# Superjomn/TiPS

Measured on AMD Instinct MI355X. Metric: device-resident fp32 bucket-sum GiB/s (% HBM peak); allreduce GiB/s 1/2/4/8 GPU, higher is better.
Workload: dtype f32

## Files before the change

### tips_amd/csrc/mxfp8.cc

```cpp
#include <algorithm>
#include <vector>

#include "mxfp8.h"
#include "rt.h"
#include "side.h"

using namespace tips::rt;

namespace {

const char kTakes[] = "the MXFP8 calls take";

struct Flat {
  int64_t elems = 0, total = 0;
  std::vector<tips::MxSeg> segs;
};

int flat_of(const void* const* ptrs, const int64_t* counts, int n, bool cover, Flat* f) {
  if (n > 0 && !ptrs) return fail(TIPS_ERR_INVALID_ARG, "bad tensor list (n %d)", n);
  TRY(check_counts(counts, n, "tensor", &f->total));
  if (f->total == 0) return 0;
  std::vector<int64_t> offs((size_t)n);
  f->elems = fused_layout(counts, n, TIPS_FLOAT32, offs.data()) / 4;
  for (int i = 0; i < n; i++)
    if (counts[i] > 0) {
      if (!ptrs[i]) return fail(TIPS_ERR_INVALID_ARG, "null pointer (tensor %d)", i);
      if ((reinterpret_cast<uintptr_t>(ptrs[i]) & 3) != 0) return fail(TIPS_ERR_INVALID_ARG, "tensor %d is not 4-B aligned", i);
      f->segs.push_back(tips::MxSeg{ptrs[i], offs[i] / 4, counts[i], (counts[i] + 31) / 32 * 32});
    }
  std::sort(f->segs.begin(), f->segs.end(), [](const tips::MxSeg& a, const tips::MxSeg& b) { return a.off < b.off; });
  if (cover) tips::mxfp8_cover(f->segs, tips::mxfp8_scales_offset(f->elems));
  return 0;
}
// ... 5 lines not shown
}

int quantize_into(const Flat& f, unsigned char* wire, float* residual, hipStream_t s) {
  const int64_t so = tips::mxfp8_scales_offset(f.elems);
  const int64_t tail_begin = so / tips::kMxBlock, tail_end = tips::mxfp8_wire_bytes(f.elems) - so;
  HIP_TRY(tips::launch_mxfp8_quantize(f.segs.data(), (int)f.segs.size(), wire, wire + so, residual, tail_begin, tail_end, s));
  return 0;
}

int64_t ef_sender_elems(int64_t E) { return tips::mxfp8_scales_offset(E); }
int64_t ef_elems(int64_t E, int p) {
  const int64_t per = p > 1 ? chunk_of(tips::mxfp8_blocks(E), p, 8, 0).len() : 0;
  return ef_sender_elems(E) + tips::kMxBlock * per;
}

bool overlaps(const void* a, int64_t an, const void* b, int64_t bn) {
  const uintptr_t x = reinterpret_cast<uintptr_t>(a), y = reinterpret_cast<uintptr_t>(b);
  return an > 0 && bn > 0 && x < y + (uintptr_t)bn && y < x + (uintptr_t)an;
}

int check_residual(const void* r, int64_t bytes, const char* what, const Flat* a, const Flat* b) {
  TRY(need_device(r, what, kTakes));
  if ((reinterpret_cast<uintptr_t>(r) & 15) != 0) return fail(TIPS_ERR_INVALID_ARG, "%s must be 16-B aligned", what);
  for (const Flat* f : {a, b})
    if (f)
      for (const tips::MxSeg& sg : f->segs)
        if (sg.ptr && overlaps(r, bytes, sg.ptr, sg.count * 4)) return fail(TIPS_ERR_INVALID_ARG, "%s overlaps a tensor of the list", what);
  return 0;
}

int dequantize_from(const Flat& f, const unsigned char* wire, double factor, hipStream_t s) {
  HIP_TRY(tips::launch_mxfp8_dequantize(f.segs.data(), (int)f.segs.size(), wire, wire + tips::mxfp8_scales_offset(f.elems),
                                        (float)factor, s));
  return 0;
}

int at_most_max_srcs(const char* what, int size) {
  if (size > tips::kMxMaxSrcs)
    return fail(TIPS_ERR_UNSUPPORTED, "%s folds at most %d ranks, not %d", what, tips::kMxMaxSrcs, size);
  return 0;
}

int agree(int size, int n, int64_t total, const int64_t* counts, int own, bool with_ef) {
  const uint64_t h = hash_counts(counts, n);
  const int64_t mine[4] = {n, total, (int64_t)(with_ef ? (h ^ 0xEFull) * kFnvPrime : h), own};
  SideRecords rec;
  TRY(side_exchange(size, mine, 4, &rec));
  if (const int r = rec.first_differing(0, 3); r >= 0) {
    const int64_t *q = rec.of(r), *q0 = rec.of(0);
    return fail(TIPS_ERR_MISMATCH,
                "Mismatched MXFP8 allreduce: rank %d has %lld tensors, %lld elements, count hash %llx; rank 0 has %lld "
                "tensors, %lld elements, count hash %llx",
                r, (long long)q[0], (long long)q[1], (unsigned long long)q[2], (long long)q0[0], (long long)q0[1],
                (unsigned long long)q0[2]);
  }
  if (!own) TRY(rec.report_refusing("MXFP8 allreduce"));
  return rec.report_own();
}

struct Part {
  unsigned char *payload, *scales;
  int64_t blocks;
};

template <class To, class From>
int exchange(State& st, hipStream_t s, To&& to, From&& from) {
  TRY(rccl_enter(st, s));
  NCCL_TRY(ncclGroupStart());
  for (int q = 0; q < st.size; q++) {
    if (q == st.rank) continue;
    const Part t = to(q), f = from(q);
    if (t.blocks > 0) {
      NCCL_TRY(ncclSend(t.payload, (size_t)(t.blocks * tips::kMxBlock), ncclInt8, q, st.comm, s));
      NCCL_TRY(ncclSend(t.scales, (size_t)t.blocks, ncclInt8, q, st.comm, s));
    }
    if (f.blocks > 0) {
      NCCL_TRY(ncclRecv(f.payload, (size_t)(f.blocks * tips::kMxBlock), ncclInt8, q, st.comm, s));
      NCCL_TRY(ncclRecv(f.scales, (size_t)f.blocks, ncclInt8, q, st.comm, s));
    }
  }
  NCCL_TRY(ncclGroupEnd());
  return rccl_leave(st, s);
}

int run_collective(State& st, const Flat& in, const Flat& out, double factor, float* ef, hipStream_t s) {
  const int p = st.size, rank = st.rank;
  const int64_t E = in.elems, B = tips::mxfp8_blocks(E), so = tips::mxfp8_scales_offset(E);
  const int64_t wire = tips::mxfp8_wire_bytes(E);
  const int64_t per = p > 1 ? chunk_of(B, p, 8, 0).len() : 0;
  const int64_t slot = round_up(per * tips::kMxBlock + per, kAlignBytes);
  TRY(st.mxfp8.open(s, (size_t)(2 * wire + (p - 1) * slot)));
  unsigned char* w0 = (unsigned char*)st.mxfp8.scratch.p;
  unsigned char* w1 = w0 + wire;
  unsigned char* stage = w1 + wire;
  TRY(quantize_into(in, w0, ef, s));
  const unsigned char* reduced = w0;
  if (p > 1) {
    TRY(ensure_comm(st));
    auto slot_of = [&](int r) { return stage + (int64_t)(r < rank ? r : r - 1) * slot; };
    auto staged = [&](int r, int64_t blocks) { return Part{slot_of(r), slot_of(r) + per * tips::kMxBlock, blocks}; };
    auto blocks_of = [&](unsigned char* w, Range c) { return Part{w + c.b * tips::kMxBlock, w + so + c.b, c.len()}; };
    const Range mine = chunk_of(B, p, 8, rank);
    TRY(exchange(
        st, s, [&](int q) { return blocks_of(w0, chunk_of(B, p, 8, q)); }, [&](int q) { return staged(q, mine.len()); }));
    if (mine.len() > 0) {
      tips::MxSrcs srcs = {};
      for (int r = 0; r < p; r++) {
        const Part src = r == rank ? blocks_of(w0, mine) : staged(r, mine.len());
        srcs.payload[r] = src.payload;
        srcs.scales[r] = src.scales;
      }
      const Part dst = blocks_of(w1, mine);
      HIP_TRY(tips::launch_mxfp8_fold(dst.payload, dst.scales, srcs, p, mine.len(), ef ? ef + ef_sender_elems(E) : nullptr, s));
    }
    TRY(exchange(
        st, s, [&](int) { return blocks_of(w1, mine); }, [&](int q) { return blocks_of(w1, chunk_of(B, p, 8, q)); }));
    reduced = w1;
  }
  TRY(dequantize_from(out, reduced, factor, s));
  return st.mxfp8.close(s);
}

int collective(const char* what, const void* const* ins, const int64_t* counts, int n, void* const* outs, double factor,
               bool with_ef, void* ef, int64_t ef_bytes, hipStream_t s) {
  TRY(check_factor(factor));
  Flat in, out;
  TRY(flat_of(ins, counts, n, true, &in));
  TRY(flat_of(outs, counts, n, false, &out));
  State& st = S();
  std::unique_lock<std::mutex> one;
  int size;
  TRY(side_open(st, st.mxfp8, what, "MXFP8", at_most_max_srcs, true, &one, &size));
  int own = refuse_capture(what, s);
  for (size_t i = 0; i < in.segs.size() && own == 0; i++)
    if (in.segs[i].ptr) own = need_device(in.segs[i].ptr, "an input", kTakes);
  for (size_t i = 0; i < out.segs.size() && own == 0; i++) own = need_device(out.segs[i].ptr, "an output", kTakes);
  if (with_ef && in.total > 0 && own == 0) {
    const int64_t need = 4 * ef_elems(in.elems, size);
    if (ef_bytes < need)
      own = fail(TIPS_ERR_MISMATCH, "%s: ef_bytes %lld is below tips_mxfp8_ef_bytes(%lld, %d) = %lld", what, (long long)ef_bytes,
                 (long long)in.elems, size, (long long)need);
    else own = check_residual(ef, need, "ef", &in, &out);
  }
  TRY(agree(size, n, in.total, counts, own, with_ef));
  if (in.total == 0) return 0;
  std::lock_guard<std::mutex> lk(st.mu);
  if (!st.initialized) return fail(TIPS_ERR_NOT_INITIALIZED, "tips_init has not been called");
  TRY(set_device(st));
  return run_collective(st, in, out, factor, with_ef ? (float*)ef : nullptr, s);
}

int fold_blocks(void* dst_wire, const void* const* src_wires, int nsrc, int64_t flat_elems, int64_t block_begin,
                int64_t block_count, bool with_ef, void* residual, hipStream_t s) {
  if (nsrc < 1 || nsrc > tips::kMxMaxSrcs) return fail(TIPS_ERR_INVALID_ARG, "nsrc must be 1 ... %d (got %d)", tips::kMxMaxSrcs, nsrc);
  if (flat_elems < 0 || flat_elems > ((int64_t)1 << 56) || block_begin < 0 || block_count < 0)
    return fail(TIPS_ERR_INVALID_ARG, "negative size (elements %lld, blocks %lld + %lld)", (long long)flat_elems,
                (long long)block_begin, (long long)block_count);
  if (block_count > tips::mxfp8_blocks(flat_elems) - block_begin)
    return fail(TIPS_ERR_INVALID_ARG, "blocks %lld + %lld lie outside the buffer's %lld", (long long)block_begin,
                (long long)block_count, (long long)tips::mxfp8_blocks(flat_elems));
  if (!src_wires) return fail(TIPS_ERR_INVALID_ARG, "null pointer (src_wires)");
  if (block_count == 0) return 0;
  TRY(check_wire(dst_wire, "dst_wire"));
  const int64_t so = tips::mxfp8_scales_offset(flat_elems);
  tips::MxSrcs srcs = {};
  for (int j = 0; j < nsrc; j++) {
    TRY(check_wire(src_wires[j], "a source wire buffer"));
    srcs.payload[j] = (const unsigned char*)src_wires[j] + block_begin * tips::kMxBlock;
    srcs.scales[j] = (const unsigned char*)src_wires[j] + so + block_begin;
  }
  if (with_ef) {
    const int64_t rbytes = 4 * tips::kMxBlock * block_count, wbytes = tips::mxfp8_wire_bytes(flat_elems);
    TRY(check_residual(residual, rbytes, "residual", nullptr, nullptr));
    bool hit = overlaps(residual, rbytes, dst_wire, wbytes);
    for (int j = 0; j < nsrc; j++) hit = hit || overlaps(residual, rbytes, src_wires[j], wbytes);
    if (hit) return fail(TIPS_ERR_INVALID_ARG, "residual overlaps a wire buffer");
  }
  unsigned char* d = (unsigned char*)dst_wire;
  HIP_TRY(tips::launch_mxfp8_fold(d + block_begin * tips::kMxBlock, d + so + block_begin, srcs, nsrc, block_count,
                                  with_ef ? (float*)residual : nullptr, s));
  return 0;
}

int flat_collective(const char* what, const void* const* ins, const int64_t* counts, int n, void* flat, double factor,
                    bool with_ef, void* ef, int64_t ef_bytes, hipStream_t s) {
  if (n < 0 || (n > 0 && (!counts || !ins))) return fail(TIPS_ERR_INVALID_ARG, "bad tensor list (n %d)", n);
  std::vector<int64_t> offs((size_t)n);
  std::vector<void*> outs((size_t)n, nullptr);
  int64_t total;
  TRY(check_counts(counts, n, "tensor", &total));
  if (total > 0) {
    if (!flat) return fail(TIPS_ERR_INVALID_ARG, "null pointer (flat)");
    fused_layout(counts, n, TIPS_FLOAT32, offs.data());
    for (int i = 0; i < n; i++)
      if (counts[i] > 0) outs[i] = (char*)flat + offs[i];
  }
  return collective(what, ins, counts, n, outs.data(), factor, with_ef, ef, ef_bytes, s);
}

}

extern "C" {

int64_t tips_mxfp8_wire_bytes(int64_t flat_elems, int64_t* scales_offset) {
  if (flat_elems < 0 || flat_elems > ((int64_t)1 << 56)) return fail(TIPS_ERR_INVALID_ARG, "bad size (%lld elements)", (long long)flat_elems);
  if (scales_offset) *scales_offset = tips::mxfp8_scales_offset(flat_elems);
  return tips::mxfp8_wire_bytes(flat_elems);
}

int tips_mxfp8_quantize(const void* const* ins, const int64_t* counts, int n, void* wire, void* stream) {
  Flat f;
  TRY(flat_of(ins, counts, n, true, &f));
  if (f.total == 0) return 0;
  TRY(check_wire(wire, "wire"));
  for (const tips::MxSeg& sg : f.segs)
    if (sg.ptr) TRY(need_device(sg.ptr, "a tensor of the list", kTakes));
  return quantize_into(f, (unsigned char*)wire, nullptr, (hipStream_t)stream);
}

int64_t tips_mxfp8_ef_bytes(int64_t flat_elems, int nranks) {
  if (flat_elems < 0 || flat_elems > ((int64_t)1 << 56)) return fail(TIPS_ERR_INVALID_ARG, "bad size (%lld elements)", (long long)flat_elems);
  if (nranks < 1 || nranks > tips::kMxMaxSrcs) return fail(TIPS_ERR_INVALID_ARG, "nranks must be 1 ... %d (got %d)", tips::kMxMaxSrcs, nranks);
  return 4 * ef_elems(flat_elems, nranks);
}

int tips_mxfp8_quantize_ef(const void* const* ins, const int64_t* counts, int n, void* wire, void* residual, void* stream) {
  Flat f;
  TRY(flat_of(ins, counts, n, true, &f));
  if (f.total == 0) return 0;
  TRY(check_wire(wire, "wire"));
  for (const tips::MxSeg& sg : f.segs)
    if (sg.ptr) TRY(need_device(sg.ptr, "a tensor of the list", kTakes));
  const int64_t rbytes = 4 * ef_sender_elems(f.elems);
  TRY(check_residual(residual, rbytes, "residual", &f, nullptr));
  if (overlaps(residual, rbytes, wire, tips::mxfp8_wire_bytes(f.elems))) return fail(TIPS_ERR_INVALID_ARG, "residual overlaps the wire buffer");
  return quantize_into(f, (unsigned char*)wire, (float*)residual, (hipStream_t)stream);
}

int tips_mxfp8_fold(void* dst_wire, const void* const* src_wires, int nsrc, int64_t flat_elems, int64_t block_begin,
                    int64_t block_count, void* stream) {
  return fold_blocks(dst_wire, src_wires, nsrc, flat_elems, block_begin, block_count, false, nullptr, (hipStream_t)stream);
}

int tips_mxfp8_fold_ef(void* dst_wire, const void* const* src_wires, int nsrc, int64_t flat_elems, int64_t block_begin,
                       int64_t block_count, void* residual, void* stream) {
  return fold_blocks(dst_wire, src_wires, nsrc, flat_elems, block_begin, block_count, true, residual, (hipStream_t)stream);
}

int tips_mxfp8_dequantize(void* const* outs, const int64_t* counts, int n, const void* wire, double factor, void* stream) {
  TRY(check_factor(factor));
  Flat f;
  TRY(flat_of(outs, counts, n, false, &f));
  if (f.total == 0) return 0;
  TRY(check_wire(wire, "wire"));
  for (const tips::MxSeg& sg : f.segs) TRY(need_device(sg.ptr, "a tensor of the list", kTakes));
  return dequantize_from(f, (const unsigned char*)wire, factor, (hipStream_t)stream);
}

int tips_allreduce_mxfp8(const void* in, void* out, int64_t count, double factor, void* stream) {
  if (count < 0) return fail(TIPS_ERR_INVALID_ARG, "negative count");
  return collective("tips_allreduce_mxfp8", &in, &count, 1, &out, factor, false, nullptr, 0, (hipStream_t)stream);
}

int tips_allreduce_mxfp8_ef(const void* in, void* out, int64_t count, double factor, void* ef, int64_t ef_bytes, void* stream) {
  if (count < 0) return fail(TIPS_ERR_INVALID_ARG, "negative count");
  return collective("tips_allreduce_mxfp8_ef", &in, &count, 1, &out, factor, true, ef, ef_bytes, (hipStream_t)stream);
}

int tips_fused_allreduce_mxfp8_flat(const void* const* ins, const int64_t* counts, int n, void* flat, double factor,
                                    void* stream) {
  return flat_collective("tips_fused_allreduce_mxfp8_flat", ins, counts, n, flat, factor, false, nullptr, 0, (hipStream_t)stream);
}

int tips_fused_allreduce_mxfp8_ef_flat(const void* const* ins, const int64_t* counts, int n, void* flat, double factor,
                                       void* ef, int64_t ef_bytes, void* stream) {
  return flat_collective("tips_fused_allreduce_mxfp8_ef_flat", ins, counts, n, flat, factor, true, ef, ef_bytes,
                         (hipStream_t)stream);
}

}
```

### tips_amd/csrc/mxfp8.h

```cpp
#pragma once

#include <hip/hip_runtime.h>
#include <stdint.h>

#include <vector>

namespace tips {

constexpr int kMxBlock = 32;
inline int64_t mxfp8_blocks(int64_t elems) { return (elems + kMxBlock - 1) / kMxBlock; }
inline int64_t mxfp8_scales_offset(int64_t elems) { return (elems + 255) / 256 * 256; }
inline int64_t mxfp8_wire_bytes(int64_t elems) { return mxfp8_scales_offset(elems) + (mxfp8_blocks(elems) + 255) / 256 * 256; }

struct MxSeg {
  const void* ptr;
  int64_t off, count, span;
};
constexpr int kMxSegsPerLaunch = 48;
constexpr int64_t kMxTileElems = 4096;

inline void mxfp8_cover(std::vector<MxSeg>& segs, int64_t end) {
  for (size_t i = 0; i < segs.size(); i++) segs[i].span = (i + 1 < segs.size() ? segs[i + 1].off : end) - segs[i].off;
  if (segs[0].off > 0) segs.insert(segs.begin(), MxSeg{nullptr, 0, 0, segs[0].off});
}

hipError_t launch_mxfp8_quantize(const MxSeg* segs, int nseg, unsigned char* payload, unsigned char* scales,
                                 float* residual, int64_t tail_begin, int64_t tail_end, hipStream_t s);
constexpr int kMxMaxSrcs = 16;
struct MxSrcs {
  const unsigned char* payload[kMxMaxSrcs];
  const unsigned char* scales[kMxMaxSrcs];
};
hipError_t launch_mxfp8_fold(unsigned char* dst_payload, unsigned char* dst_scales, const MxSrcs& srcs, int nsrc,
                             int64_t nblocks, float* residual, hipStream_t s);
hipError_t launch_mxfp8_dequantize(const MxSeg* segs, int nseg, const unsigned char* payload, const unsigned char* scales,
                                   float factor, hipStream_t s);

struct MxFoldSeg {
  const void* own;
  void* dst;
  int64_t off, count;
};
constexpr int kMxFoldSegsPerLaunch = 80;
hipError_t launch_mxfp8_fold_segs(const MxFoldSeg* segs, int nseg, const MxSrcs& wires, int nsrc, int own_pos, float factor,
                                  hipStream_t s);

}
```

### tips_amd/csrc/mxfp8.hip

```cpp
#include <type_traits>
#include <vector>

#include "kernels_device.h"
#include "mxfp8.h"
#include "reducescatter.h"

namespace tips {

namespace {

constexpr int kMxRounds = 4;
static_assert(kMxTileElems == (int64_t)kBlock * kMxRounds * 4, "a tile is 256 lanes x 4 rounds x 4 elements");
constexpr unsigned kInfBits = 0x7f800000u, kQuietNaN = 0x7fc00000u, kMax448 = 0x43e00000u;

typedef short s16x2 __attribute__((ext_vector_type(2)));
typedef float f32x2 __attribute__((ext_vector_type(2)));

struct MxSegList {
  MxSeg seg[kMxSegsPerLaunch];
  int64_t tile0[kMxSegsPerLaunch + 1];
  int nseg;
};

__device__ __forceinline__ unsigned max8(unsigned v) {
// ... 16 lines not shown
__device__ __forceinline__ float scaled_clamped(float x, float mul) {
#pragma clang fp contract(off)
  const unsigned b = __builtin_bit_cast(unsigned, x * mul);
  return __builtin_bit_cast(float, min(b & 0x7fffffffu, kMax448) | (b & 0x80000000u));
}

__device__ __forceinline__ unsigned encode4(f32x4 x, unsigned sb) {
  const float mul = __builtin_bit_cast(float, (254u - sb) << 23);
  int w = __builtin_amdgcn_cvt_pk_fp8_f32(scaled_clamped(x[0], mul), scaled_clamped(x[1], mul), 0, false);
  w = __builtin_amdgcn_cvt_pk_fp8_f32(scaled_clamped(x[2], mul), scaled_clamped(x[3], mul), w, true);
  return (unsigned)w;
}

__device__ __forceinline__ unsigned abs_max4(f32x4 x) {
  const u32x4 b = __builtin_bit_cast(u32x4, x) & 0x7fffffffu;
  return max(max(b[0], b[1]), max(b[2], b[3]));
}

__device__ __forceinline__ float scale_value(unsigned sb) {
  return __builtin_bit_cast(float, sb == 255u ? kQuietNaN : (sb ? (sb << 23) : 0x00400000u));
}

template <class List>
__device__ __forceinline__ int seg_of_tile(const List& L, int64_t t) {
  int lo = 0, hi = L.nseg - 1;
  while (lo < hi) {
    const int mid = (lo + hi + 1) >> 1;
    if (L.tile0[mid] <= t) lo = mid;
    else hi = mid - 1;
  }
  return lo;
}

template <bool HI>
__device__ __forceinline__ f32x2 decode2(unsigned w, float scale) {
#pragma clang fp contract(off)
  return __builtin_amdgcn_cvt_pk_f32_fp8((int)w, HI) * scale;
}

__device__ __forceinline__ f32x4 residual4(f32x4 c, unsigned w, unsigned sb) {
#pragma clang fp contract(off)
  const float scale = scale_value(sb);
  const f32x2 lo = decode2<false>(w, scale), hi = decode2<true>(w, scale);
  return f32x4{c[0] - lo[0], c[1] - lo[1], c[2] - hi[0], c[3] - hi[1]};
}


template <bool EF>
__device__ __forceinline__ void quantize_tile(const MxSegList& L, unsigned char* __restrict__ payload,
                                              unsigned char* __restrict__ scales, float* __restrict__ residual,
                                              int64_t tail_begin, int64_t tail_end) {
#pragma clang fp contract(off)
  const int tid = threadIdx.x;
  if (blockIdx.x == 0)
    for (int64_t j = tail_begin + tid; j < tail_end; j += kBlock) scales[j] = 0;
  const int64_t t = blockIdx.x;
  const int si = seg_of_tile(L, t);
  const MxSeg sg = L.seg[si];
  const int64_t base = (t - L.tile0[si]) * kMxTileElems;
  const float* src = (const float*)sg.ptr;
  float* res = nullptr;
  if constexpr (EF) res = residual + sg.off;
  const bool vec = (reinterpret_cast<uintptr_t>(src) & 15) == 0;
  f32x4 x[kMxRounds], r[kMxRounds];
#pragma unroll
  for (int u = 0; u < kMxRounds; u++) {
    const int64_t i0 = base + ((int64_t)u * kBlock + tid) * 4;
    x[u] = f32x4{0.f, 0.f, 0.f, 0.f};
    if constexpr (EF) {
      r[u] = f32x4{0.f, 0.f, 0.f, 0.f};
      if (i0 + 4 <= sg.count) {
        r[u] = __builtin_bit_cast(f32x4, ld16<true>((const u32x4*)(res + i0)));
        if (vec) {
          x[u] = __builtin_bit_cast(f32x4, ld16<true>((const u32x4*)(src + i0)));
        } else {
#pragma unroll
          for (int j = 0; j < 4; j++) x[u][j] = src[i0 + j];
        }
      } else if (i0 < sg.count) {
#pragma unroll
        for (int j = 0; j < 4; j++)
          if (i0 + j < sg.count) x[u][j] = src[i0 + j], r[u][j] = res[i0 + j];
      }
    } else {
      if (vec && i0 + 4 <= sg.count) {
        x[u] = __builtin_bit_cast(f32x4, ld16<true>((const u32x4*)(src + i0)));
      } else if (i0 < sg.count) {
#pragma unroll
        for (int j = 0; j < 4; j++)
          if (i0 + j < sg.count) x[u][j] = src[i0 + j];
      }
    }
  }
#pragma unroll
  for (int u = 0; u < kMxRounds; u++) {
    const int64_t i0 = base + ((int64_t)u * kBlock + tid) * 4;
    f32x4 c = x[u];
    if constexpr (EF) c = x[u] + r[u];
    const unsigned am = max8(abs_max4(c));
    if (i0 >= sg.span) continue;
    const bool poisoned = am >= kInfBits;
    const unsigned sb = poisoned ? 255u : scale_byte(am);
    const unsigned w = poisoned ? 0x7f7f7f7fu : encode4(c, sb);
    *(unsigned*)(payload + sg.off + i0) = w;
    if ((tid & 7) == 0) scales[(sg.off + i0) >> 5] = (unsigned char)sb;
    if constexpr (EF) {
      if (i0 >= sg.count) continue;
      const f32x4 rn = poisoned ? f32x4{0.f, 0.f, 0.f, 0.f} : residual4(c, w, sb);
      if (i0 + 4 <= sg.count) {
        st16<true>((u32x4*)(res + i0), __builtin_bit_cast(u32x4, rn));
      } else {
#pragma unroll
        for (int j = 0; j < 4; j++)
          if (i0 + j < sg.count) res[i0 + j] = rn[j];
      }
    }
  }
}

__global__ __launch_bounds__(kBlock) void mxfp8_quantize_kernel(MxSegList L, unsigned char* __restrict__ payload,
                                                                unsigned char* __restrict__ scales, int64_t tail_begin,
                                                                int64_t tail_end) {
  quantize_tile<false>(L, payload, scales, nullptr, tail_begin, tail_end);
}

__global__ __launch_bounds__(kBlock) void mxfp8_quantize_ef_kernel(MxSegList L, unsigned char* __restrict__ payload,
                                                                   unsigned char* __restrict__ scales,
                                                                   float* __restrict__ residual, int64_t tail_begin,
                                                                   int64_t tail_end) {
  quantize_tile<true>(L, payload, scales, residual, tail_begin, tail_end);
}

#ifndef TIPS_MXFP8_FOLD_EF_NT_LOAD
#define TIPS_MXFP8_FOLD_EF_NT_LOAD 0
#endif
#ifndef TIPS_MXFP8_FOLD_EF_NT_STORE
#define TIPS_MXFP8_FOLD_EF_NT_STORE 0
#endif
constexpr bool kFoldEfNtLoad = TIPS_MXFP8_FOLD_EF_NT_LOAD, kFoldEfNtStore = TIPS_MXFP8_FOLD_EF_NT_STORE;
template <bool EF>
__device__ __forceinline__ void fold_lane(unsigned char* dst_payload, unsigned char* dst_scales, const MxSrcs& srcs, int nsrc,
                                          int64_t nblocks, float* residual) {
#pragma clang fp contract(off)
  const int64_t g = (int64_t)blockIdx.x * kBlock + threadIdx.x;
  const int64_t blk = g >> 1;
  const bool active = blk < nblocks;
  float acc[16];
  f32x4 o[4];
#pragma unroll
  for (int j = 0; j < 16; j++) acc[j] = 0.f;
#pragma unroll
  for (int q = 0; q < 4; q++) o[q] = f32x4{0.f, 0.f, 0.f, 0.f};
  u32x4* og = nullptr;
  if constexpr (EF) og = (u32x4*)residual + g * 4;
  if (active) {
    u32x4 v = ld16<true>((const u32x4*)srcs.payload[0] + g);
    unsigned sb = srcs.scales[0][blk];
    if constexpr (EF) {
#pragma unroll
      for (int q = 0; q < 4; q++) o[q] = __builtin_bit_cast(f32x4, ld16<kFoldEfNtLoad>(og + q));
    }
    for (int k = 0; k < nsrc; k++) {
      const u32x4 cur = v;
// ... 32 lines not shown
  }
  am = max2(am);
  if (!active) return;
  const bool poisoned = am >= kInfBits;
  const unsigned sb = poisoned ? 255u : scale_byte(am);
  u32x4 w;
#pragma unroll
  for (int q = 0; q < 4; q++) {
    w[q] = poisoned ? 0x7f7f7f7fu : encode4(c[q], sb);
    if constexpr (EF) {
      const f32x4 on = poisoned ? f32x4{0.f, 0.f, 0.f, 0.f} : residual4(c[q], w[q], sb);
      st16<kFoldEfNtStore>(og + q, __builtin_bit_cast(u32x4, on));
    }
  }
  st16<false>((u32x4*)dst_payload + g, w);
  if ((g & 1) == 0) dst_scales[blk] = (unsigned char)sb;
}

__global__ __launch_bounds__(kBlock) void mxfp8_fold_kernel(unsigned char* dst_payload, unsigned char* dst_scales,
                                                            MxSrcs srcs, int nsrc, int64_t nblocks) {
  fold_lane<false>(dst_payload, dst_scales, srcs, nsrc, nblocks, nullptr);
}

__global__ __launch_bounds__(kBlock) void mxfp8_fold_ef_kernel(unsigned char* dst_payload, unsigned char* dst_scales,
                                                               MxSrcs srcs, int nsrc, int64_t nblocks,
                                                               float* __restrict__ residual) {
  fold_lane<true>(dst_payload, dst_scales, srcs, nsrc, nblocks, residual);
}

__device__ __forceinline__ float canonical(float y) {
  return y != y ? __builtin_bit_cast(float, kQuietNaN) : y;
}

__global__ __launch_bounds__(kBlock) void mxfp8_dequantize_kernel(MxSegList L, const unsigned char* __restrict__ payload,
                                                                  const unsigned char* __restrict__ scales, float factor,
                                                                  int has_factor) {
#pragma clang fp contract(off)
  const int tid = threadIdx.x;
  const int64_t t = blockIdx.x;
  const int si = seg_of_tile(L, t);
  const MxSeg sg = L.seg[si];
  const int64_t base = (t - L.tile0[si]) * kMxTileElems;
  float* dst = (float*)const_cast<void*>(sg.ptr);
  const bool vec = (reinterpret_cast<uintptr_t>(dst) & 15) == 0;
  unsigned w[kMxRounds], sb[kMxRounds];
#pragma unroll
  for (int u = 0; u < kMxRounds; u++) {
    const int64_t i0 = base + ((int64_t)u * kBlock + tid) * 4;
    w[u] = 0, sb[u] = 0;
    if (i0 < sg.count) {
      w[u] = *(const unsigned*)(payload + sg.off + i0);
      sb[u] = scales[(sg.off + i0) >> 5];
    }
  }
#pragma unroll
  for (int u = 0; u < kMxRounds; u++) {
    const int64_t i0 = base + ((int64_t)u * kBlock + tid) * 4;
    if (i0 >= sg.count) continue;
    const float scale = scale_value(sb[u]);
    const f32x2 lo = __builtin_amdgcn_cvt_scalef32_pk_f32_fp8((int)w[u], scale, false);
    const f32x2 hi = __builtin_amdgcn_cvt_scalef32_pk_f32_fp8((int)w[u], scale, true);
    f32x4 y = {lo[0], lo[1], hi[0], hi[1]};
    if (has_factor) y = y * factor;
#pragma unroll
    for (int j = 0; j < 4; j++) y[j] = canonical(y[j]);
    if (vec && i0 + 4 <= sg.count) {
      st16<false>((u32x4*)(dst + i0), __builtin_bit_cast(u32x4, y));
    } else {
#pragma unroll
      for (int j = 0; j < 4; j++)
        if (i0 + j < sg.count) dst[i0 + j] = y[j];
    }
  }
}

struct MxFoldList {
  MxFoldSeg seg[kMxFoldSegsPerLaunch];
  int64_t tile0[kMxFoldSegsPerLaunch + 1];
  MxSrcs srcs;
  int nseg, nsrc, own_pos;
};

constexpr int kMxFoldExact = 8;

template <int K>
__global__ __launch_bounds__(kBlock) void mxfp8_fold_segs_kernel(MxFoldList L, float factor, int has_factor) {
#pragma clang fp contract(off)
  constexpr bool kExact = K <= kMxFoldExact;
  constexpr int kUnroll = kExact ? kMxRounds : 1;
  const int nsrc = kExact ? K : L.nsrc;
  const int own_pos = L.own_pos;
  const int tid = threadIdx.x;
  const int64_t t = blockIdx.x;
  const int si = seg_of_tile(L, t);
  const MxFoldSeg sg = L.seg[si];
  const int64_t base = (t - L.tile0[si]) * kMxTileElems;
  const float* own = (const float*)sg.own;
  float* dst = (float*)sg.dst;
  const bool vec_own = (reinterpret_cast<uintptr_t>(own) & 15) == 0, vec_dst = (reinterpret_cast<uintptr_t>(dst) & 15) == 0;
#pragma unroll kUnroll
  for (int u = 0; u < kMxRounds; u++) {
    const int64_t i0 = base + ((int64_t)u * kBlock + tid) * 4;
    if (i0 >= sg.count) continue;
    const bool full = i0 + 4 <= sg.count;
    f32x4 x = {0.f, 0.f, 0.f, 0.f};
    if (vec_own && full) {
// ... 53 lines not shown
    for (; i < nseg && L.nseg < kCap; i++) {
      const int64_t elems = cover(segs[i]);
      if (elems <= 0) continue;
      L.seg[L.nseg] = segs[i];
      L.tile0[L.nseg++] = tiles;
      tiles += (elems + kMxTileElems - 1) / kMxTileElems;
    }
    if (!L.nseg) break;
    L.tile0[L.nseg] = tiles;
    if (tiles > 0x7fffffff) return hipErrorInvalidValue;
    const hipError_t err = launch(L, (unsigned)tiles);
    if (err != hipSuccess) return err;
  }
  return hipSuccess;
}

}

hipError_t launch_mxfp8_quantize(const MxSeg* segs, int nseg, unsigned char* payload, unsigned char* scales,
                                 float* residual, int64_t tail_begin, int64_t tail_end, hipStream_t s) {
  if (!segs || nseg < 1 || !payload || !scales) return hipErrorInvalidValue;
  MxSegList L;
  return for_each_part(L, segs, nseg, [](const MxSeg& sg) { return sg.span; }, [&](const MxSegList& part, unsigned tiles) {
    if (residual)
      hipLaunchKernelGGL(mxfp8_quantize_ef_kernel, dim3(tiles), dim3(kBlock), 0, s, part, payload, scales, residual,
                         tail_begin, tail_end);
    else
      hipLaunchKernelGGL(mxfp8_quantize_kernel, dim3(tiles), dim3(kBlock), 0, s, part, payload, scales, tail_begin, tail_end);
    tail_begin = tail_end = 0;
    return hipGetLastError();
  });
}

hipError_t launch_mxfp8_fold(unsigned char* dst_payload, unsigned char* dst_scales, const MxSrcs& srcs, int nsrc,
                             int64_t nblocks, float* residual, hipStream_t s) {
  if (!dst_payload || !dst_scales || nsrc < 1 || nsrc > kMxMaxSrcs || nblocks < 0) return hipErrorInvalidValue;
  if (nblocks == 0) return hipSuccess;
  const int64_t grid = (2 * nblocks + kBlock - 1) / kBlock;
  if (grid > 0x7fffffff) return hipErrorInvalidValue;
  if (residual)
    hipLaunchKernelGGL(mxfp8_fold_ef_kernel, dim3((unsigned)grid), dim3(kBlock), 0, s, dst_payload, dst_scales, srcs, nsrc,
                       nblocks, residual);
  else
    hipLaunchKernelGGL(mxfp8_fold_kernel, dim3((unsigned)grid), dim3(kBlock), 0, s, dst_payload, dst_scales, srcs, nsrc,
                       nblocks);
  return hipGetLastError();
}

hipError_t launch_mxfp8_dequantize(const MxSeg* segs, int nseg, const unsigned char* payload, const unsigned char* scales,
                                   float factor, hipStream_t s) {
  if (!segs || nseg < 1 || !payload || !scales) return hipErrorInvalidValue;
  MxSegList L;
  return for_each_part(L, segs, nseg, [](const MxSeg& sg) { return sg.count; }, [&](const MxSegList& part, unsigned tiles) {
    hipLaunchKernelGGL(mxfp8_dequantize_kernel, dim3(tiles), dim3(kBlock), 0, s, part, payload, scales, factor,
                       factor != 1.0f ? 1 : 0);
    return hipGetLastError();
  });
}

hipError_t launch_mxfp8_fold_segs(const MxFoldSeg* segs, int nseg, const MxSrcs& wires, int nsrc, int own_pos, float factor,
                                  hipStream_t s) {
  if (nseg < 0 || (nseg > 0 && !segs) || nsrc < 1 || nsrc > kMxMaxSrcs || own_pos < 0 || own_pos >= nsrc)
    return hipErrorInvalidValue;
  if (nsrc == 1) {
    std::vector<FoldSeg> plain;
    for (int i = 0; i < nseg; i++)
// ... 23 lines not shown
```

Baseline: 6299.

## Cache device tile tables for large MXFP8 tensor lists in single launches

Tensor lists with more segments than fit in one launch's kernel argument now get a per-tile descriptor table. The table is built on the host, uploaded to device memory once, and kept in a 16-entry LRU keyed by pointers and counts. Quantize and dequantize then run as one tiles-indexed launch instead of several chunked launches, which cuts launch and host setup overhead on repeated calls. This adds stream-ordering bookkeeping, an H2D copy when a table misses, and per-block loads of the descriptors. The measured fp32 bucket-sum and allreduce paths likely never touch MXFP8.

```diff
diff --git a/tips_amd/csrc/mxfp8.cc b/tips_amd/csrc/mxfp8.cc
--- a/tips_amd/csrc/mxfp8.cc
+++ b/tips_amd/csrc/mxfp8.cc
@@ -1,4 +1,7 @@
+#include <string.h>
+
 #include <algorithm>
+#include <mutex>
 #include <vector>
 
 #include "mxfp8.h"
@@ -70,6 +73,171 @@
 int dequantize_from(const Flat& f, const unsigned char* wire, double factor, hipStream_t s) {
   HIP_TRY(tips::launch_mxfp8_dequantize(f.segs.data(), (int)f.segs.size(), wire, wire + tips::mxfp8_scales_offset(f.elems),
                                         (float)factor, s));
+  return 0;
+}
+
+struct TileTable {
+  Flat flat;
+  tips::MxTile* dev = nullptr;
+  size_t cap = 0;
+  int64_t ntiles = 0;
+  hipEvent_t ev_up = nullptr;
+  std::vector<hipStream_t> readers;
+};
+
+struct TableStore {
+  std::mutex mu;
+  tips::MxLru lru[2];
+  TileTable tab[2][tips::kMxTables];
+  void* host = nullptr;
+  size_t host_cap = 0;
+  hipEvent_t ev_host = nullptr;
+  hipEvent_t ev_order = nullptr;
+};
+
+TableStore& table_store() {
+  static TableStore* ts = new TableStore();
+  return *ts;
+}
+
+bool is_capturing(hipStream_t s) {
+  hipStreamCaptureStatus cs = hipStreamCaptureStatusNone;
+  if (hipStreamIsCapturing(s, &cs) != hipSuccess) {
+    (void)hipGetLastError();
+    return false;
+  }
+  return cs != hipStreamCaptureStatusNone;
+}
+
+int settle(TableStore& ts, TileTable& t, hipStream_t s) {
+  if (!ts.ev_order) HIP_TRY(hipEventCreateWithFlags(&ts.ev_order, hipEventDisableTiming));
+  for (hipStream_t r : t.readers) {
+    if (r == s) continue;
+    hipError_t e = hipEventRecord(ts.ev_order, r);
+    if (e == hipSuccess) e = hipStreamWaitEvent(s, ts.ev_order, 0);
+    if (e != hipSuccess) {
+      (void)hipGetLastError();
+      HIP_TRY(hipDeviceSynchronize());
+      break;
+    }
+  }
+  t.readers.clear();
+  return 0;
+}
+
+int fill_table(TableStore& ts, TileTable& t, int kind, Flat&& f, hipStream_t s) {
+  std::vector<tips::MxTile> tiles;
+  const int64_t ntiles = tips::mxfp8_build_tiles(f.segs.data(), (int)f.segs.size(),
+                                                 kind == tips::kMxQuantizeTable ? tips::kMxCoverSpan : tips::kMxCoverCount, &tiles);
+  if (ntiles < 1 || ntiles > 0x7fffffff) HIP_TRY(hipErrorInvalidValue);
+  const size_t bytes = (size_t)ntiles * sizeof(tips::MxTile);
+  TRY(settle(ts, t, s));
+  t.ntiles = 0;
+  if (t.cap < (size_t)ntiles) {
+    if (t.dev) HIP_TRY(hipFree(t.dev));
+    t.dev = nullptr;
+    t.cap = 0;
+    const size_t cap = std::max<size_t>((size_t)ntiles, 1024);
+    HIP_TRY(hipMalloc((void**)&t.dev, cap * sizeof(tips::MxTile)));
+    t.cap = cap;
+  }
+  if (ts.ev_host) HIP_TRY(hipEventSynchronize(ts.ev_host));
+  if (ts.host_cap < bytes) {
+    if (ts.host) HIP_TRY(hipHostFree(ts.host));
+    ts.host = nullptr;
+    ts.host_cap = 0;
+    const size_t cap = std::max<size_t>(bytes, 256 << 10);
+    HIP_TRY(hipHostMalloc(&ts.host, cap, hipHostMallocDefault));
+    ts.host_cap = cap;
+  }
+  if (!t.ev_up) HIP_TRY(hipEventCreateWithFlags(&t.ev_up, hipEventDisableTiming));
+  memcpy(ts.host, tiles.data(), bytes);
+  HIP_TRY(hipMemcpyAsync(t.dev, ts.host, bytes, hipMemcpyHostToDevice, s));
+  t.readers.push_back(s);
+  HIP_TRY(hipEventRecord(t.ev_up, s));
+  ts.ev_host = t.ev_up;
+  t.flat = std::move(f);
+  t.ntiles = ntiles;
+  return 0;
+}
+
+struct ListOperand {
+  const Flat* f = nullptr;
+  TileTable* t = nullptr;
+  Flat own;
+  std::unique_lock<std::mutex> lock;
+};
+
+bool list_may_have_table(const void* const* ptrs, const int64_t* counts, int n, hipStream_t s) {
+  return ptrs && counts && n >= tips::kMxSegsPerLaunch && !is_capturing(s);
+}
+
+int table_of(int kind, const void* const* ptrs, const int64_t* counts, int n, const Flat& f, hipStream_t s,
+             std::unique_lock<std::mutex>& lock, ListOperand* op) {
+  op->f = &f;
+  if ((int)f.segs.size() <= tips::kMxSegsPerLaunch) return 0;
+  TableStore& ts = table_store();
+  if (!lock.owns_lock()) lock = std::unique_lock<std::mutex>(ts.mu);
+  int i = ts.lru[kind].find(kind, ptrs, counts, n);
+  if (i < 0) {
+    bool evicted;
+    i = ts.lru[kind].take(kind, ptrs, counts, n, &evicted);
+    Flat copy = f;
+    const int rc = fill_table(ts, ts.tab[kind][i], kind, std::move(copy), s);
+    if (rc != 0) {
+      ts.lru[kind].drop(i);
+      return rc;
+    }
+  }
+  op->t = &ts.tab[kind][i];
+  return 0;
+}
+
+int local_operand(int kind, const void* const* ptrs, const int64_t* counts, int n, const void* wire, hipStream_t s,
+                  ListOperand* op) {
+  const bool may = list_may_have_table(ptrs, counts, n, s);
+  if (may) {
+    TableStore& ts = table_store();
+    op->lock = std::unique_lock<std::mutex>(ts.mu);
+    const int i = ts.lru[kind].find(kind, ptrs, counts, n);
+    if (i >= 0) {
+      op->t = &ts.tab[kind][i];
+      op->f = &op->t->flat;
+      return check_wire(wire, "wire");
+    }
+  }
+  op->f = &op->own;
+  TRY(flat_of(ptrs, counts, n, kind == tips::kMxQuantizeTable, &op->own));
+  if (op->own.total == 0) return 0;
+  TRY(check_wire(wire, "wire"));
+  for (const tips::MxSeg& sg : op->own.segs)
+    if (sg.ptr) TRY(need_device(sg.ptr, "a tensor of the list", kTakes));
+  if (!may) return 0;
+  return table_of(kind, ptrs, counts, n, op->own, s, op->lock, op);
+}
+
+int join_readers(TileTable& t, hipStream_t s) {
+  if (std::find(t.readers.begin(), t.readers.end(), s) != t.readers.end()) return 0;
+  HIP_TRY(hipStreamWaitEvent(s, t.ev_up, 0));
+  if (t.readers.size() >= 16) TRY(settle(table_store(), t, s));
+  t.readers.push_back(s);
+  return 0;
+}
+
+int quantize_list(const ListOperand& op, unsigned char* wire, float* residual, hipStream_t s) {
+  if (!op.t) return quantize_into(*op.f, wire, residual, s);
+  const int64_t so = tips::mxfp8_scales_offset(op.f->elems);
+  TRY(join_readers(*op.t, s));
+  HIP_TRY(tips::launch_mxfp8_quantize_tiles(op.t->dev, op.t->ntiles, wire, wire + so, residual, so / tips::kMxBlock,
+                                            tips::mxfp8_wire_bytes(op.f->elems) - so, s));
+  return 0;
+}
+
+int dequantize_list(const ListOperand& op, const unsigned char* wire, double factor, hipStream_t s) {
+  if (!op.t) return dequantize_from(*op.f, wire, factor, s);
+  TRY(join_readers(*op.t, s));
+  HIP_TRY(tips::launch_mxfp8_dequantize_tiles(op.t->dev, op.t->ntiles, wire, wire + tips::mxfp8_scales_offset(op.f->elems),
+                                              (float)factor, s));
   return 0;
 }
 
@@ -121,9 +289,9 @@
   return rccl_leave(st, s);
 }
 
-int run_collective(State& st, const Flat& in, const Flat& out, double factor, float* ef, hipStream_t s) {
+int run_collective(State& st, const ListOperand& in, const ListOperand& out, double factor, float* ef, hipStream_t s) {
   const int p = st.size, rank = st.rank;
-  const int64_t E = in.elems, B = tips::mxfp8_blocks(E), so = tips::mxfp8_scales_offset(E);
+  const int64_t E = in.f->elems, B = tips::mxfp8_blocks(E), so = tips::mxfp8_scales_offset(E);
   const int64_t wire = tips::mxfp8_wire_bytes(E);
   const int64_t per = p > 1 ? chunk_of(B, p, 8, 0).len() : 0;
   const int64_t slot = round_up(per * tips::kMxBlock + per, kAlignBytes);
@@ -131,7 +299,7 @@
   unsigned char* w0 = (unsigned char*)st.mxfp8.scratch.p;
   unsigned char* w1 = w0 + wire;
   unsigned char* stage = w1 + wire;
-  TRY(quantize_into(in, w0, ef, s));
+  TRY(quantize_list(in, w0, ef, s));
   const unsigned char* reduced = w0;
   if (p > 1) {
     TRY(ensure_comm(st));
@@ -155,7 +323,7 @@
         st, s, [&](int) { return blocks_of(w1, mine); }, [&](int q) { return blocks_of(w1, chunk_of(B, p, 8, q)); }));
     reduced = w1;
   }
-  TRY(dequantize_from(out, reduced, factor, s));
+  TRY(dequantize_list(out, reduced, factor, s));
   return st.mxfp8.close(s);
 }
 
@@ -185,7 +353,10 @@
   std::lock_guard<std::mutex> lk(st.mu);
   if (!st.initialized) return fail(TIPS_ERR_NOT_INITIALIZED, "tips_init has not been called");
   TRY(set_device(st));
-  return run_collective(st, in, out, factor, with_ef ? (float*)ef : nullptr, s);
+  ListOperand qin, qout;
+  TRY(table_of(tips::kMxQuantizeTable, ins, counts, n, in, s, qin.lock, &qin));
+  TRY(table_of(tips::kMxDequantizeTable, outs, counts, n, out, s, qin.lock, &qout));
+  return run_collective(st, qin, qout, factor, with_ef ? (float*)ef : nullptr, s);
 }
 
 int fold_blocks(void* dst_wire, const void* const* src_wires, int nsrc, int64_t flat_elems, int64_t block_begin,
@@ -247,13 +418,10 @@
 }
 
 int tips_mxfp8_quantize(const void* const* ins, const int64_t* counts, int n, void* wire, void* stream) {
-  Flat f;
-  TRY(flat_of(ins, counts, n, true, &f));
-  if (f.total == 0) return 0;
-  TRY(check_wire(wire, "wire"));
-  for (const tips::MxSeg& sg : f.segs)
-    if (sg.ptr) TRY(need_device(sg.ptr, "a tensor of the list", kTakes));
-  return quantize_into(f, (unsigned char*)wire, nullptr, (hipStream_t)stream);
+  ListOperand op;
+  TRY(local_operand(tips::kMxQuantizeTable, ins, counts, n, wire, (hipStream_t)stream, &op));
+  if (op.f->total == 0) return 0;
+  return quantize_list(op, (unsigned char*)wire, nullptr, (hipStream_t)stream);
 }
 
 int64_t tips_mxfp8_ef_bytes(int64_t flat_elems, int nranks) {
@@ -263,16 +431,14 @@
 }
 
 int tips_mxfp8_quantize_ef(const void* const* ins, const int64_t* counts, int n, void* wire, void* residual, void* stream) {
-  Flat f;
-  TRY(flat_of(ins, counts, n, true, &f));
-  if (f.total == 0) return 0;
-  TRY(check_wire(wire, "wire"));
-  for (const tips::MxSeg& sg : f.segs)
-    if (sg.ptr) TRY(need_device(sg.ptr, "a tensor of the list", kTakes));
+  ListOperand op;
+  TRY(local_operand(tips::kMxQuantizeTable, ins, counts, n, wire, (hipStream_t)stream, &op));
+  if (op.f->total == 0) return 0;
+  const Flat& f = *op.f;
   const int64_t rbytes = 4 * ef_sender_elems(f.elems);
   TRY(check_residual(residual, rbytes, "residual", &f, nullptr));
   if (overlaps(residual, rbytes, wire, tips::mxfp8_wire_bytes(f.elems))) return fail(TIPS_ERR_INVALID_ARG, "residual overlaps the wire buffer");
-  return quantize_into(f, (unsigned char*)wire, (float*)residual, (hipStream_t)stream);
+  return quantize_list(op, (unsigned char*)wire, (float*)residual, (hipStream_t)stream);
 }
 
 int tips_mxfp8_fold(void* dst_wire, const void* const* src_wires, int nsrc, int64_t flat_elems, int64_t block_begin,
@@ -287,12 +453,10 @@
 
 int tips_mxfp8_dequantize(void* const* outs, const int64_t* counts, int n, const void* wire, double factor, void* stream) {
   TRY(check_factor(factor));
-  Flat f;
-  TRY(flat_of(outs, counts, n, false, &f));
-  if (f.total == 0) return 0;
-  TRY(check_wire(wire, "wire"));
-  for (const tips::MxSeg& sg : f.segs) TRY(need_device(sg.ptr, "a tensor of the list", kTakes));
-  return dequantize_from(f, (const unsigned char*)wire, factor, (hipStream_t)stream);
+  ListOperand op;
+  TRY(local_operand(tips::kMxDequantizeTable, outs, counts, n, wire, (hipStream_t)stream, &op));
+  if (op.f->total == 0) return 0;
+  return dequantize_list(op, (const unsigned char*)wire, factor, (hipStream_t)stream);
 }
 
 int tips_allreduce_mxfp8(const void* in, void* out, int64_t count, double factor, void* stream) {
diff --git a/tips_amd/csrc/mxfp8.h b/tips_amd/csrc/mxfp8.h
--- a/tips_amd/csrc/mxfp8.h
+++ b/tips_amd/csrc/mxfp8.h
@@ -4,6 +4,8 @@
 #include <stdint.h>
 
 #include <vector>
+
+#include "mxfp8_table.h"
 
 namespace tips {
 
@@ -12,12 +14,7 @@
 inline int64_t mxfp8_scales_offset(int64_t elems) { return (elems + 255) / 256 * 256; }
 inline int64_t mxfp8_wire_bytes(int64_t elems) { return mxfp8_scales_offset(elems) + (mxfp8_blocks(elems) + 255) / 256 * 256; }
 
-struct MxSeg {
-  const void* ptr;
-  int64_t off, count, span;
-};
 constexpr int kMxSegsPerLaunch = 48;
-constexpr int64_t kMxTileElems = 4096;
 
 inline void mxfp8_cover(std::vector<MxSeg>& segs, int64_t end) {
   for (size_t i = 0; i < segs.size(); i++) segs[i].span = (i + 1 < segs.size() ? segs[i + 1].off : end) - segs[i].off;
@@ -35,6 +32,10 @@
                              int64_t nblocks, float* residual, hipStream_t s);
 hipError_t launch_mxfp8_dequantize(const MxSeg* segs, int nseg, const unsigned char* payload, const unsigned char* scales,
                                    float factor, hipStream_t s);
+hipError_t launch_mxfp8_quantize_tiles(const MxTile* tiles, int64_t ntiles, unsigned char* payload, unsigned char* scales,
+                                       float* residual, int64_t tail_begin, int64_t tail_end, hipStream_t s);
+hipError_t launch_mxfp8_dequantize_tiles(const MxTile* tiles, int64_t ntiles, const unsigned char* payload,
+                                         const unsigned char* scales, float factor, hipStream_t s);
 
 struct MxFoldSeg {
   const void* own;
diff --git a/tips_amd/csrc/mxfp8.hip b/tips_amd/csrc/mxfp8.hip
--- a/tips_amd/csrc/mxfp8.hip
+++ b/tips_amd/csrc/mxfp8.hip
@@ -72,6 +72,13 @@
   return lo;
 }
 
+template <class List>
+__device__ __forceinline__ MxTile list_tile(const List& L, MxCover c) {
+  const int64_t t = blockIdx.x;
+  const int si = seg_of_tile(L, t);
+  return mxfp8_tile_of(L.seg[si], (t - L.tile0[si]) * kMxTileElems, c);
+}
+
 template <bool HI>
 __device__ __forceinline__ f32x2 decode2(unsigned w, float scale) {
 #pragma clang fp contract(off)
@@ -87,25 +94,21 @@
 
 
 template <bool EF>
-__device__ __forceinline__ void quantize_tile(const MxSegList& L, unsigned char* __restrict__ payload,
+__device__ __forceinline__ void quantize_tile(const MxTile sg, unsigned char* __restrict__ payload,
                                               unsigned char* __restrict__ scales, float* __restrict__ residual,
                                               int64_t tail_begin, int64_t tail_end) {
 #pragma clang fp contract(off)
   const int tid = threadIdx.x;
   if (blockIdx.x == 0)
     for (int64_t j = tail_begin + tid; j < tail_end; j += kBlock) scales[j] = 0;
-  const int64_t t = blockIdx.x;
-  const int si = seg_of_tile(L, t);
-  const MxSeg sg = L.seg[si];
-  const int64_t base = (t - L.tile0[si]) * kMxTileElems;
   const float* src = (const float*)sg.ptr;
   float* res = nullptr;
-  if constexpr (EF) res = residual + sg.off;
+  if constexpr (EF) res = residual + sg.pos;
   const bool vec = (reinterpret_cast<uintptr_t>(src) & 15) == 0;
   f32x4 x[kMxRounds], r[kMxRounds];
 #pragma unroll
   for (int u = 0; u < kMxRounds; u++) {
-    const int64_t i0 = base + ((int64_t)u * kBlock + tid) * 4;
+    const int64_t i0 = ((int64_t)u * kBlock + tid) * 4;
     x[u] = f32x4{0.f, 0.f, 0.f, 0.f};
     if constexpr (EF) {
       r[u] = f32x4{0.f, 0.f, 0.f, 0.f};
@@ -134,7 +137,7 @@
   }
 #pragma unroll
   for (int u = 0; u < kMxRounds; u++) {
-    const int64_t i0 = base + ((int64_t)u * kBlock + tid) * 4;
+    const int64_t i0 = ((int64_t)u * kBlock + tid) * 4;
     f32x4 c = x[u];
     if constexpr (EF) c = x[u] + r[u];
     const unsigned am = max8(abs_max4(c));
@@ -142,8 +145,8 @@
     const bool poisoned = am >= kInfBits;
     const unsigned sb = poisoned ? 255u : scale_byte(am);
     const unsigned w = poisoned ? 0x7f7f7f7fu : encode4(c, sb);
-    *(unsigned*)(payload + sg.off + i0) = w;
-    if ((tid & 7) == 0) scales[(sg.off + i0) >> 5] = (unsigned char)sb;
+    *(unsigned*)(payload + sg.pos + i0) = w;
+    if ((tid & 7) == 0) scales[(sg.pos + i0) >> 5] = (unsigned char)sb;
     if constexpr (EF) {
       if (i0 >= sg.count) continue;
       const f32x4 rn = poisoned ? f32x4{0.f, 0.f, 0.f, 0.f} : residual4(c, w, sb);
@@ -161,14 +164,29 @@
 __global__ __launch_bounds__(kBlock) void mxfp8_quantize_kernel(MxSegList L, unsigned char* __restrict__ payload,
                                                                 unsigned char* __restrict__ scales, int64_t tail_begin,
                                                                 int64_t tail_end) {
-  quantize_tile<false>(L, payload, scales, nullptr, tail_begin, tail_end);
+  quantize_tile<false>(list_tile(L, kMxCoverSpan), payload, scales, nullptr, tail_begin, tail_end);
+}
+
+__global__ __launch_bounds__(kBlock) void mxfp8_quantize_tiles_kernel(const MxTile* __restrict__ tiles,
+                                                                      unsigned char* __restrict__ payload,
+                                                                      unsigned char* __restrict__ scales, int64_t tail_begin,
+                                                                      int64_t tail_end) {
+  quantize_tile<false>(tiles[blockIdx.x], payload, scales, nullptr, tail_begin, tail_end);
+}
+
+__global__ __launch_bounds__(kBlock) void mxfp8_quantize_ef_tiles_kernel(const MxTile* __restrict__ tiles,
+                                                                         unsigned char* __restrict__ payload,
+                                                                         unsigned char* __restrict__ scales,
+                                                                         float* __restrict__ residual, int64_t tail_begin,
+                                                                         int64_t tail_end) {
+  quantize_tile<true>(tiles[blockIdx.x], payload, scales, residual, tail_begin, tail_end);
 }
 
 __global__ __launch_bounds__(kBlock) void mxfp8_quantize_ef_kernel(MxSegList L, unsigned char* __restrict__ payload,
                                                                    unsigned char* __restrict__ scales,
                                                                    float* __restrict__ residual, int64_t tail_begin,
                                                                    int64_t tail_end) {
-  quantize_tile<true>(L, payload, scales, residual, tail_begin, tail_end);
+  quantize_tile<true>(list_tile(L, kMxCoverSpan), payload, scales, residual, tail_begin, tail_end);
 }
 
 #ifndef TIPS_MXFP8_FOLD_EF_NT_LOAD
@@ -267,30 +285,25 @@
   return y != y ? __builtin_bit_cast(float, kQuietNaN) : y;
 }
 
-__global__ __launch_bounds__(kBlock) void mxfp8_dequantize_kernel(MxSegList L, const unsigned char* __restrict__ payload,
-                                                                  const unsigned char* __restrict__ scales, float factor,
-                                                                  int has_factor) {
+__device__ __forceinline__ void dequantize_tile(const MxTile sg, const unsigned char* __restrict__ payload,
+                                                const unsigned char* __restrict__ scales, float factor, int has_factor) {
 #pragma clang fp contract(off)
   const int tid = threadIdx.x;
-  const int64_t t = blockIdx.x;
-  const int si = seg_of_tile(L, t);
-  const MxSeg sg = L.seg[si];
-  const int64_t base = (t - L.tile0[si]) * kMxTileElems;
   float* dst = (float*)const_cast<void*>(sg.ptr);
   const bool vec = (reinterpret_cast<uintptr_t>(dst) & 15) == 0;
   unsigned w[kMxRounds], sb[kMxRounds];
 #pragma unroll
   for (int u = 0; u < kMxRounds; u++) {
-    const int64_t i0 = base + ((int64_t)u * kBlock + tid) * 4;
+    const int64_t i0 = ((int64_t)u * kBlock + tid) * 4;
     w[u] = 0, sb[u] = 0;
     if (i0 < sg.count) {
-      w[u] = *(const unsigned*)(payload + sg.off + i0);
-      sb[u] = scales[(sg.off + i0) >> 5];
+      w[u] = *(const unsigned*)(payload + sg.pos + i0);
+      sb[u] = scales[(sg.pos + i0) >> 5];
     }
   }
 #pragma unroll
   for (int u = 0; u < kMxRounds; u++) {
-    const int64_t i0 = base + ((int64_t)u * kBlock + tid) * 4;
+    const int64_t i0 = ((int64_t)u * kBlock + tid) * 4;
     if (i0 >= sg.count) continue;
     const float scale = scale_value(sb[u]);
     const f32x2 lo = __builtin_amdgcn_cvt_scalef32_pk_f32_fp8((int)w[u], scale, false);
@@ -307,6 +320,19 @@
         if (i0 + j < sg.count) dst[i0 + j] = y[j];
     }
   }
+}
+
+__global__ __launch_bounds__(kBlock) void mxfp8_dequantize_kernel(MxSegList L, const unsigned char* __restrict__ payload,
+                                                                  const unsigned char* __restrict__ scales, float factor,
+                                                                  int has_factor) {
+  dequantize_tile(list_tile(L, kMxCoverCount), payload, scales, factor, has_factor);
+}
+
+__global__ __launch_bounds__(kBlock) void mxfp8_dequantize_tiles_kernel(const MxTile* __restrict__ tiles,
+                                                                        const unsigned char* __restrict__ payload,
+                                                                        const unsigned char* __restrict__ scales, float factor,
+                                                                        int has_factor) {
+  dequantize_tile(tiles[blockIdx.x], payload, scales, factor, has_factor);
 }
 
 struct MxFoldList {
@@ -426,6 +452,26 @@
   });
 }
 
+hipError_t launch_mxfp8_quantize_tiles(const MxTile* tiles, int64_t ntiles, unsigned char* payload, unsigned char* scales,
+                                       float* residual, int64_t tail_begin, int64_t tail_end, hipStream_t s) {
+  if (!tiles || ntiles < 1 || ntiles > 0x7fffffff || !payload || !scales) return hipErrorInvalidValue;
+  if (residual)
+    hipLaunchKernelGGL(mxfp8_quantize_ef_tiles_kernel, dim3((unsigned)ntiles), dim3(kBlock), 0, s, tiles, payload, scales,
+                       residual, tail_begin, tail_end);
+  else
+    hipLaunchKernelGGL(mxfp8_quantize_tiles_kernel, dim3((unsigned)ntiles), dim3(kBlock), 0, s, tiles, payload, scales,
+                       tail_begin, tail_end);
+  return hipGetLastError();
+}
+
+hipError_t launch_mxfp8_dequantize_tiles(const MxTile* tiles, int64_t ntiles, const unsigned char* payload,
+                                         const unsigned char* scales, float factor, hipStream_t s) {
+  if (!tiles || ntiles < 1 || ntiles > 0x7fffffff || !payload || !scales) return hipErrorInvalidValue;
+  hipLaunchKernelGGL(mxfp8_dequantize_tiles_kernel, dim3((unsigned)ntiles), dim3(kBlock), 0, s, tiles, payload, scales, factor,
+                     factor != 1.0f ? 1 : 0);
+  return hipGetLastError();
+}
+
 hipError_t launch_mxfp8_fold(unsigned char* dst_payload, unsigned char* dst_scales, const MxSrcs& srcs, int nsrc,
                              int64_t nblocks, float* residual, hipStream_t s) {
   if (!dst_payload || !dst_scales || nsrc < 1 || nsrc > kMxMaxSrcs || nblocks < 0) return hipErrorInvalidValue;
diff --git a/tips_amd/csrc/mxfp8_table.cc b/tips_amd/csrc/mxfp8_table.cc
--- /dev/null
+++ b/tips_amd/csrc/mxfp8_table.cc
@@ -0,0 +1,71 @@
+#include "mxfp8_table.h"
+
+#include <algorithm>
+
+namespace tips {
+
+int64_t mxfp8_build_tiles(const MxSeg* segs, int nseg, MxCover c, std::vector<MxTile>* tiles) {
+  int64_t total = 0;
+  for (int i = 0; i < nseg; i++) {
+    const int64_t elems = mxfp8_covered(segs[i], c);
+    if (elems > 0) total += (elems + kMxTileElems - 1) / kMxTileElems;
+  }
+  tiles->clear();
+  tiles->reserve((size_t)total);
+  for (int i = 0; i < nseg; i++) {
+    const int64_t elems = mxfp8_covered(segs[i], c);
+    for (int64_t base = 0; base < elems; base += kMxTileElems) tiles->push_back(mxfp8_tile_of(segs[i], base, c));
+  }
+  return total;
+}
+
+uint64_t mxfp8_key_hash(int kind, const void* const* ptrs, const int64_t* counts, int n) {
+  constexpr uint64_t kBasis = 0xcbf29ce484222325ull, kPrime = 0x100000001b3ull;
+  uint64_t h = (kBasis ^ (uint64_t)kind) * kPrime;
+  h = (h ^ (uint64_t)n) * kPrime;
+  for (int i = 0; i < n; i++) {
+    h = (h ^ (uint64_t)reinterpret_cast<uintptr_t>(ptrs[i])) * kPrime;
+    h = (h ^ (uint64_t)counts[i]) * kPrime;
+  }
+  return h;
+}
+
+void MxKey::assign(int kind_, const void* const* p, const int64_t* c, int n) {
+  kind = kind_;
+  hash = mxfp8_key_hash(kind_, p, c, n);
+  ptrs.assign(p, p + n);
+  counts.assign(c, c + n);
+}
+
+bool MxKey::matches(int kind_, uint64_t hash_, const void* const* p, const int64_t* c, int n) const {
+  return kind == kind_ && hash == hash_ && (int)ptrs.size() == n && std::equal(ptrs.begin(), ptrs.end(), p) &&
+         std::equal(counts.begin(), counts.end(), c);
+}
+
+int MxLru::find(int kind, const void* const* ptrs, const int64_t* counts, int n) {
+  const uint64_t h = mxfp8_key_hash(kind, ptrs, counts, n);
+  for (int i = 0; i < kMxTables; i++)
+    if (slot[i].used && slot[i].key.matches(kind, h, ptrs, counts, n)) {
+      slot[i].stamp = ++clock;
+      return i;
+    }
+  return -1;
+}
+
+int MxLru::take(int kind, const void* const* ptrs, const int64_t* counts, int n, bool* evicted) {
+  int at = -1;
+  for (int i = 0; i < kMxTables && at < 0; i++)
+    if (!slot[i].used) at = i;
+  *evicted = at < 0;
+  if (at < 0) {
+    at = 0;
+    for (int i = 1; i < kMxTables; i++)
+      if (slot[i].stamp < slot[at].stamp) at = i;
+  }
+  slot[at].key.assign(kind, ptrs, counts, n);
+  slot[at].used = true;
+  slot[at].stamp = ++clock;
+  return at;
+}
+
+}
diff --git a/tips_amd/csrc/mxfp8_table.h b/tips_amd/csrc/mxfp8_table.h
--- /dev/null
+++ b/tips_amd/csrc/mxfp8_table.h
@@ -0,0 +1,65 @@
+#pragma once
+
+#include <stdint.h>
+
+#include <vector>
+
+#ifdef __HIPCC__
+#define TIPS_MX_HD __host__ __device__
+#else
+#define TIPS_MX_HD
+#endif
+
+namespace tips {
+
+struct MxSeg {
+  const void* ptr;
+  int64_t off, count, span;
+};
+constexpr int64_t kMxTileElems = 4096;
+
+struct MxTile {
+  const void* ptr;
+  int64_t pos, count, span;
+};
+static_assert(sizeof(MxTile) == 32, "a tile record is one 32-B load");
+
+enum MxCover { kMxCoverSpan = 0, kMxCoverCount = 1 };
+TIPS_MX_HD inline int64_t mxfp8_covered(const MxSeg& sg, MxCover c) { return c == kMxCoverSpan ? sg.span : sg.count; }
+
+TIPS_MX_HD inline MxTile mxfp8_tile_of(const MxSeg& sg, int64_t base, MxCover c) {
+  const int64_t left = sg.count > base ? sg.count - base : 0;
+  return MxTile{left > 0 ? (const void*)((const float*)sg.ptr + base) : nullptr, sg.off + base, left,
+                mxfp8_covered(sg, c) - base};
+}
+
+int64_t mxfp8_build_tiles(const MxSeg* segs, int nseg, MxCover c, std::vector<MxTile>* tiles);
+
+enum MxKind { kMxQuantizeTable = 0, kMxDequantizeTable = 1 };
+
+struct MxKey {
+  int kind = 0;
+  uint64_t hash = 0;
+  std::vector<const void*> ptrs;
+  std::vector<int64_t> counts;
+  void assign(int kind_, const void* const* p, const int64_t* c, int n);
+  bool matches(int kind_, uint64_t hash_, const void* const* p, const int64_t* c, int n) const;
+};
+uint64_t mxfp8_key_hash(int kind, const void* const* ptrs, const int64_t* counts, int n);
+
+constexpr int kMxTables = 16;
+
+struct MxLru {
+  struct Slot {
+    MxKey key;
+    bool used = false;
+    uint64_t stamp = 0;
+  };
+  Slot slot[kMxTables];
+  uint64_t clock = 0;
+  int find(int kind, const void* const* ptrs, const int64_t* counts, int n);
+  int take(int kind, const void* const* ptrs, const int64_t* counts, int n, bool* evicted);
+  void drop(int i) { slot[i].used = false; }
+};
+
+}
```

Measured after the change: 6175. -2.0%, worse.
